# TakiRyo/object-triggered-3D-SLAM

Measured on AMD Instinct MI355X. Metric: RGB-D frames/sec (640×480, 5mm voxel TSDF) at 1/2/4/8 GPU; Mpoints/s filtered, higher is better.
Workload: dtype f32 tsdf/weight + f64 colour; 1 GPU; configs[1]: 256-frame 640x480 RGB-D TSDF integration, 5 mm voxel, sdf_trunc 0.04, one object scan per GPU (synthetic box-on-floor ring scan), colour precision 64 (Open3D's float64 TSDFVoxel::color_, exact division: bit-exact colours); color_precision=64, width=640, height=480, volume_units=5896, parallelism=objects1

## Files before the change

object-triggered-3d-slam_amd/_lib.py:

```python
from __future__ import annotations

import ctypes as C
import os
import threading

_HERE = os.path.dirname(os.path.abspath(__file__))
LIB_PATH = os.path.join(_HERE, "libotslam_hip.so")
HEADER_PATH = os.path.join(os.path.dirname(_HERE), "include", "otslam.h")

OT_OK = 0
OT_ERR_INVALID_ARGUMENT = 1
OT_ERR_UNSUPPORTED_FORMAT = 2
OT_ERR_CAPACITY = 3
OT_ERR_HIP = 4

OT_COLOR_NONE = 0
OT_COLOR_RGB8 = 1


class ot_intrinsics(C.Structure):
    _fields_ = [("width", C.c_int32), ("height", C.c_int32), ("fx", C.c_double), ("fy", C.c_double),
                ("cx", C.c_double), ("cy", C.c_double)]


# ... 123 lines not shown
class OTError(RuntimeError):
    """Raised for any non-OK status; message mirrors Open3D's utility::LogError text."""


TEST_SIGNATURES = {
    "otx_serial_chain_f64": [_p, _i64, _i32, _p, _pi64, _p],
    "otx_chain_walk_trace": [_p, _i64, _i32, _p, _p, _i32, _p],
    "otx_tsdf_stats": [_p, _p],
    "otx_unit_sort_radix": [_i32],
    "otx_sor_netfill": [_i32],
    "otx_integrate_fine": [_i32],
    "otx_integrate_workgroup": [_i32],
    "otx_touch_stage_blocks": [_i32],
    "otx_touch_frames": [_i32],
    "otx_split_frontend": [_i32],
    "otx_defer_integrate": [_i32],
    "otx_integrate_depth": [_i32],
    "otx_mc_emit_fork": [_i32],
    "otx_normals_at": [_i32],
    "otx_sampler_hi_stream": [_i32],
    "otx_sort_pairs_u64_u32": [_p, _p, _p, _p, _i64, _i32, _p],
    "otx_sort_segments_u32_u32": [_p, _p, _p, _p, _p, _i32, _i32, _p],
    "otx_alloc_count": [],
    "otx_registration_last_d2": [_p, _i64, _p],
}


def use_variant(path: str) -> None:
    global LIB_PATH
    path = os.path.abspath(path)
# ... 66 lines not shown
```

object-triggered-3d-slam_amd/csrc/tsdf.h:

```cpp
#pragma once

#include <vector>

#include "common.h"

namespace ot {

constexpr int UNIT_RES = 16;
constexpr int UNIT_VOX = UNIT_RES * UNIT_RES * UNIT_RES;
constexpr int UNIT_FIELDS = 5;
constexpr int UNIT_FLOATS = UNIT_FIELDS * UNIT_VOX;
constexpr int UNIT_FLOATS_C64 = 8 * UNIT_VOX;

constexpr int C_UNUSED0 = 0;
constexpr int C_UNITS = 1;
constexpr int C_OVERFLOW = 2;
constexpr int C_HASHERR = 3;
constexpr int C_BATCH_PAIRS = 4;
constexpr int C_ORDER_HEAVY = 6;
constexpr int C_ORDER_LIGHT = 7;
constexpr int C_KMAX = 8;
constexpr int C_KNEG = 11;
constexpr int C_UNITS_DONE = 14;
constexpr int N_COUNTERS = 16;

constexpr int S_UPDATES = 0;
constexpr int S_UNIT_INTEGRATIONS = 1;

struct TsdfDev {
    unsigned long long* hkeys;
    int* hvals;
    int* counters;
    unsigned long long* stats;
    int* unit_keys;
    float* vox;
    int unit_floats;
    int color64;
    unsigned long long* fmask;
    int* bslots;
    void* work;
    int hash_mask;
    int max_units;
// ... 110 lines not shown
};

struct IntegrateParams {
    const float* depth;
    const uint8_t* color;
    const float* mult;
    int W, H;
    float fx, fy, cx, cy;
    float E[12];
    float es0, es1, es2;
    float vl, half, trunc, trunc_inv, safe_w, safe_h;
    float inv_fx, inv_fy;
    float proj_eps;
    int rcp_hi;
    double unit_len;
};

struct BatchTouchParams {
    int W, stride, ws, hs;
    double fx, fy, cx, cy;
    double trunc, unit_len;
    double inv_unit;
    int slot_cap;
    int64_t npx;
    int pc;
    int tiles;
    int stage_blocks;
    int tf;
    int sample_stage;
};

struct StageMaskParams {
    int W, H, tiles_x, tiles_y, wpr;
    float fx, fy, cx, cy, vl, half;
    double unit_len;
    int nframes;
};

struct UnitWork {
    int id;
    int kx, ky, kz;
    unsigned long long mask;
    unsigned long long pad;
};

enum class BatchMode { Direct, Overlap, Deferred };
struct BatchPlan {
    BatchMode mode = BatchMode::Direct;
    bool split = false;
    int set = 0;
    int* wcount = nullptr;
    int* wcopy = nullptr;
};

struct BatchCtx {
    BatchPlan plan;
    BatchTouchParams tp;
    IntegrateParams ip0;
    StageMaskParams sq{};
    unsigned* smask = nullptr;
    int n, pc, variant;
};

struct PendingFrame {
// ... 47 lines not shown
    ot_intrinsics mult_intr{};
    bool mult_valid = false;
    int batch_max = ot::MAX_BATCH;
    std::vector<ot::PendingFrame> pending;
    ot::BatchFrame* hbframes = nullptr;
    unsigned* hmail = nullptr;
    int hb_next = 0;
    unsigned units_seq = 0;
    int early_frame = -1;
    unsigned mc_seq = 0;
    int batch_pc = ot::C_BATCH_PAIRS;
    struct BatchSet {
        ot::BatchFrame* bframes = nullptr;
        uint2* bdc = nullptr;
        int64_t cap = 0;
        void* work = nullptr;
        hipEvent_t ev_units = nullptr;
        hipEvent_t ev_done = nullptr;
    } bset[2];
    int overlap_mode = -1;
    unsigned* tmask = nullptr;
    int64_t tmask_words = 0;
    int tmask_w = 0, tmask_h = 0;
    int split_mode = -1;
    bool dfr_on = false;
    hipStream_t dfr_stream = nullptr;
    hipEvent_t ev_dfr = nullptr;
    ot::BatchCtx dfr;
    int64_t stat_batches = 0, stat_unit_batches = 0, stat_fresh = 0, stat_prev_units = 0;
    int64_t last_batch_slots = -1;
// ... 18 lines not shown
    std::vector<std::pair<hipEvent_t, hipEvent_t>> prof_fe_events;
    double prof_fe_ms = 0.0;
    int64_t prof_fe_batches = 0;
};

namespace ot {
struct TsdfHooks {
    int int_fine = -1;
    int fine_units = -1;
    int int_depth = -1;
    int int_wg = -1;
    int stage_blocks = -1;
    int touch_tf = -1;
    int split = -1;
    int defer = -1;
    bool unit_sort_radix = false;
};
extern TsdfHooks g_tsdf_hooks;

ot_status reserve_units(ot_tsdf* vol, int64_t extra, hipStream_t stream);
ot_status export_list(ot_tsdf* vol, hipStream_t stream, const unsigned** ids, int64_t* n);
ot_status tsdf_sorted_units(ot_tsdf* vol, hipStream_t stream, int64_t* n_units);
struct MailSrc {
    const unsigned* p[ot::OT_MAIL_WORDS];
    int n;
};
ot_status mail_words(ot_tsdf* vol, const MailSrc& s, hipStream_t stream);
ot_status mail_wait(const unsigned* word, unsigned seq, hipStream_t stream);
ot_status tsdf_flush(ot_tsdf* vol, hipStream_t stream, bool join = true);
ot_status wait_normals(ot_tsdf* vol, hipStream_t stream);
// ... 6 lines not shown
```

object-triggered-3d-slam_amd/csrc/tsdf.hip:

```cpp
#include <algorithm>
#include <cmath>
#include <cstring>
#include <type_traits>
#include <utility>

#include "tsdf.h"

namespace ot {

typedef unsigned u32x2 __attribute__((ext_vector_type(2)));

__device__ inline __amdgpu_buffer_rsrc_t make_rsrc(const void* base, int bytes) {
    return __builtin_amdgcn_make_buffer_rsrc(const_cast<void*>(base), (short)0, bytes, 0x00020000);
}

__device__ inline double ld_f64(__amdgpu_buffer_rsrc_t r, int i) {
    const u32x2 v = __builtin_amdgcn_raw_buffer_load_b64(r, i * 8, 0, 0);
    return __hiloint2double((int)v.y, (int)v.x);
}
__device__ inline void st_f64(__amdgpu_buffer_rsrc_t r, int i, double x) {
    u32x2 v;
    v.x = (unsigned)__double2loint(x);
    v.y = (unsigned)__double2hiint(x);
    __builtin_amdgcn_raw_buffer_store_b64(v, r, i * 8, 0, 0);
}
// ... 129 lines not shown
        unsigned long long k = keys[h];
        if (k == KEY_EMPTY) {
            const unsigned long long old = atomicCAS(&keys[h], KEY_EMPTY, key);
            if (old == KEY_EMPTY) used[atomicAdd(nused, 1)] = (unsigned short)h;
            k = (old == KEY_EMPTY) ? key : old;
        }
        if (k == key) {
            atomicOr(&masks[h], bit);
            return true;
        }
        h = (h + 1) & (LTAB - 1);
    }
    return false;
}

__device__ inline void stage_share(const BatchFrame* __restrict__ frames, const BatchTouchParams& p, int nframes,
                                   int grp, int part, int parts) {
    const int64_t quads = (p.npx + 3) >> 2;
    const int64_t per = (quads + parts - 1) / parts;
    const int64_t q0 = (int64_t)part * per, q1 = q0 + per < quads ? q0 + per : quads;
    for (int f = grp * p.tf; f < grp * p.tf + p.tf && f < nframes; ++f)
        prep_range(frames[f], q0 + threadIdx.x, q1, p.npx);
}

struct TouchLds {
    unsigned long long keys[LTAB];
    unsigned long long masks[LTAB];
    unsigned short used[LTAB];
    int nused;
};
template <bool REPLAY, bool STAGE = !REPLAY>
__device__ __forceinline__ void touch_body(const BatchFrame* __restrict__ frames, const BatchTouchParams& p,
                                           const TsdfDev& d, int nframes, TouchLds& L, int tile, int grp) {
    unsigned long long* s_keys = L.keys;
    unsigned long long* s_masks = L.masks;
    unsigned short* s_used = L.used;
    int& s_nused = L.nused;
// ... 552 lines not shown
        frame_tap<ZB, true>(fr, p, npx, fpx, fpy, fpz, z0, pixv, pcz, dv, cv);
        bool some = false;
#pragma unroll
        for (int k = 0; k < ZB; ++k) some |= cand[k] = voxel_candidate<true>(p, pixv[k], pcz[k], dv[k], df[k]);
        if (__builtin_amdgcn_ballot_w64(some) == 0ull) continue;
        const __amdgpu_buffer_rsrc_t mult_rsrc = make_rsrc(p.mult, npx * 4);
#pragma unroll
        for (int k = 0; k < ZB; ++k) mv[k] = voxel_multiplier<true>(mult_rsrc, pixv[k], cand[k]);
#pragma unroll
        for (int k = 0; k < ZB; ++k)
            voxel_update<C64, FAST>(cand[k], df[k] * __uint_as_float(mv[k]), cv[k], use_color, p, s_r32, s_r64, ts[k],
                                    wt[k], cr[k], cg[k], cb[k], upd);
    }
}

template <bool C64, bool FAST, int ZB, int KT>
__device__ __forceinline__ void integrate_item(const BatchFrame* __restrict__ frames, const IntegrateParams& p,
                                               const TsdfDev& d, const UnitWork& w, int s, int npx,
                                               const float* s_r32, const double* s_r64, unsigned& upd) {
    using CT = typename std::conditional<C64, double, float>::type;
    const int ent = w.id;
    const unsigned long long mask = w.mask;
    if (ent == -1) return;
    const int id = ent & 0x7FFFFFFF;
    const bool fresh = ent < 0;
    unsigned tid = threadIdx.x;
    asm volatile("" : "+v"(tid));
    const int lane = tid & 63;
    const int x = (s & 2) * 4 + (lane >> 3), y = (s & 1) * 8 + (lane & 7);
    const int col = x * 16 + y;
    const int z0 = (s >> 2) * ZB;
    float* base = d.vox + (size_t)id * (C64 ? UNIT_FLOATS_C64 : UNIT_FLOATS);
    const __amdgpu_buffer_rsrc_t col64 = make_rsrc(base + 2 * UNIT_VOX, 3 * UNIT_VOX * 8);
    float ts[ZB], wt[ZB];
    CT cr[ZB], cg[ZB], cb[ZB];
#pragma unroll
    for (int k = 0; k < ZB; ++k) {
// ... 90 lines not shown
            st_f64(col64, UNIT_VOX + vi, cg[k]);
            st_f64(col64, 2 * UNIT_VOX + vi, cb[k]);
        } else {
            base[2 * UNIT_VOX + vi] = cr[k];
            base[3 * UNIT_VOX + vi] = cg[k];
            base[4 * UNIT_VOX + vi] = cb[k];
        }
    }
}

template <bool C64, bool FAST>
struct RcpLds {
    float r32[(FAST && !C64) ? RCP_N + 1 : 1];
    double r64[(FAST && C64) ? RCP_N + 1 : 1];
};
template <bool C64, bool FAST, int ZB, int KT, bool HEAVY, int WG>
__device__ __forceinline__ void integrate_body(const BatchFrame* __restrict__ frames, const IntegrateParams& p,
                                               const TsdfDev& d, const UnitWork* __restrict__ work,
                                               const int* __restrict__ wcount, float* s_r32, double* s_r64, int bid,
                                               int nblk) {
    constexpr int PARTS = 4 * (UNIT_RES / ZB) / WG;
    {
        const int n0 = __builtin_amdgcn_readfirstlane(__hip_atomic_load(wcount, __ATOMIC_RELAXED, __HIP_MEMORY_SCOPE_AGENT));
        if (bid >= (PARTS == 1 ? n0 : ((n0 + 7) / 8) * 8 * PARTS)) return;
    }
    if constexpr (FAST) {
        for (int r = 1 + threadIdx.x; r <= p.rcp_hi; r += 64 * WG) {
            if constexpr (C64) s_r64[r] = 1.0 / (double)r;
            else s_r32[r] = 1.0f / (float)r;
        }
        if constexpr (WG > 1) __syncthreads();
        else __builtin_amdgcn_fence(__ATOMIC_ACQ_REL, "wavefront");
    }
    const int wave = __builtin_amdgcn_readfirstlane((int)(threadIdx.x >> 6));
    const int n = *wcount;
    const int nh = HEAVY ? wcount[2] : 0;
    const int npx = p.W * p.H;
    unsigned upd = 0;
    const int items = PARTS == 1 ? n : ((n + 7) / 8) * 8 * PARTS;
    for (int it = bid; it < items; it += nblk) {
        const int u = PARTS == 1 ? it : (it / (8 * PARTS)) * 8 + (it & 7);
        if (PARTS > 1 && u >= n) continue;
        const int part = PARTS == 1 ? 0 : (it >> 3) % PARTS;
        const int s = part * WG + wave;
        integrate_item<C64, FAST, ZB, KT>(frames, p, d, work[!HEAVY || u < nh ? u : n - 1 - (u - nh)], s, npx, s_r32,
                                          s_r64, upd);
    }
    const unsigned long long tot = wave_sum((unsigned long long)upd);
    if ((threadIdx.x & 63) == 0 && tot) atomicAdd(&d.stats[S_UPDATES], tot);
}

extern __shared__ double s_rcp_dyn[];
template <bool C64, bool FAST, int ZB = BZ, int KT = 1, int WG = INT_WG>
__global__ __launch_bounds__(64 * WG, (C64 && !FAST) ? 5 : (ZB == 2 ? 4 : INT_WAVES_PER_EU)) void k_batch_integrate(
    const BatchFrame* __restrict__ frames, IntegrateParams p, TsdfDev d, const UnitWork* __restrict__ work,
    const int* __restrict__ wcount) {
    integrate_body<C64, FAST, ZB, KT, false, WG>(frames, p, d, work, wcount, reinterpret_cast<float*>(s_rcp_dyn),
                                                 s_rcp_dyn, (int)blockIdx.x, (int)gridDim.x);
}

template <bool C64, bool FAST>
__global__ __launch_bounds__(64 * INT_WG, (C64 && !FAST) ? 5 : INT_WAVES_PER_EU) void k_integrate_touch(
    const BatchFrame* __restrict__ frames, IntegrateParams p, TsdfDev d, const UnitWork* __restrict__ work,
    const int* __restrict__ wcount, int nint, const BatchFrame* __restrict__ tframes, BatchTouchParams tp, int tn) {
    union Lds {
        TouchLds t;
        RcpLds<C64, FAST> r;
    };
    __shared__ Lds lds;
    const int b = (int)blockIdx.x;
    if (b < nint) {
        integrate_body<C64, FAST, BZ, 1, true, INT_WG>(frames, p, d, work, wcount, lds.r.r32, lds.r.r64, b, nint);
    } else {
// ... 37 lines not shown
    for (int k = 0; k < 16; ++k) E[k] = (float)ext[k];
    for (int k = 0; k < 12; ++k) p.E[k] = E[k];
    const double unit_voxel_length = vol->unit_length / (double)UNIT_RES;
    p.vl = (float)unit_voxel_length;
    p.half = p.vl * 0.5f;
    p.es0 = E[0 * 4 + 2] * p.vl;
    p.es1 = E[1 * 4 + 2] * p.vl;
    p.es2 = E[2 * 4 + 2] * p.vl;
    p.trunc = (float)vol->sdf_trunc;
    p.trunc_inv = 1.0f / p.trunc;
    p.safe_w = (float)in->width - 0.0001f;
    p.safe_h = (float)in->height - 0.0001f;
    p.proj_eps = (float)(std::ldexp((double)std::max(in->width, in->height) + 2.0, -21) + 1.2e-4);
    p.rcp_hi = RCP_N;
    p.unit_len = vol->unit_length;
    return p;
}

static ot_status launch_deferred(ot_tsdf* vol, hipStream_t stream, const BatchCtx* next);
static ot_status ensure_mult(ot_tsdf* vol, const ot_intrinsics* in, hipStream_t stream) {
    if (vol->mult_valid && std::memcmp(&vol->mult_intr, in, sizeof(ot_intrinsics)) == 0) return OT_OK;
    if (vol->mult) {
        ot_status sd = launch_deferred(vol, stream, nullptr);
        if (sd != OT_OK) return sd;
        if (vol->istream) OT_HIP_TRY(hipStreamSynchronize(vol->istream));
        OT_HIP_TRY(hipStreamSynchronize(stream));
        OT_HIP_TRY(hipFree(vol->mult));
        vol->mult = nullptr;
    }
    OT_HIP_TRY(hipMalloc(&vol->mult, sizeof(float) * (size_t)in->width * in->height));
// ... 240 lines not shown
    OT_HIP_TRY(hipStreamSynchronize(stream));
    for (void* p : {(void*)d.vox, (void*)d.unit_keys, (void*)vol->sorted_ids, (void*)d.hkeys, (void*)d.hvals,
                    (void*)d.fmask, (void*)d.bslots, d.work, vol->bset[1].work})
        if (p) (void)hipFree(p);
    d = nd;
    vol->bset[1].work = work1;
    vol->sorted_ids = nsorted;
    vol->max_units = nmax;
    vol->hash_cap = cap;
    return OT_OK;
}


static ot_status plan_batch(ot_tsdf* vol, const ot_intrinsics& in, int pc, BatchPlan& p) {
    p.split = split_on(vol) && tmask_fits(in.width, in.height);
    p.mode = defer_on(vol, p.split) ? BatchMode::Deferred : overlap_on(vol) ? BatchMode::Overlap : BatchMode::Direct;
    p.wcount = vol->dev.counters + pc;
    if (p.mode != BatchMode::Direct) {
        ot_status st = ensure_overlap(vol);
        if (st != OT_OK) return st;
        p.set = vol->bset_next;
        vol->bset_next ^= 1;
        p.wcount = p.wcopy = vol->wcount + p.set;
    }
    return OT_OK;
}

static void fill_batch_frames(const ot_tsdf* vol, const PendingFrame* frames, int n, uint2* bdc, int64_t npx, float vl,
                              BatchFrame* host) {
    for (int k = 0; k < n; ++k) {
// ... 19 lines not shown
    BatchTouchParams tp;
    tp.npx = (int64_t)in.width * in.height;
    tp.pc = pc;
    tp.W = in.width, tp.stride = vol->stride;
    tp.ws = (in.width + vol->stride - 1) / vol->stride;
    tp.hs = (in.height + vol->stride - 1) / vol->stride;
    tp.fx = in.fx, tp.fy = in.fy, tp.cx = in.cx, tp.cy = in.cy;
    tp.trunc = vol->sdf_trunc;
    tp.unit_len = vol->unit_length, tp.inv_unit = 1.0 / vol->unit_length;
    tp.slot_cap = (int)vol->hash_cap;
    tp.tiles = ((tp.ws + TT - 1) / TT) * ((tp.hs + TT - 1) / TT);
    tp.stage_blocks = g_tsdf_hooks.stage_blocks < 0 ? 2 * tp.tiles : g_tsdf_hooks.stage_blocks;
    tp.tf = g_tsdf_hooks.touch_tf > 0 ? g_tsdf_hooks.touch_tf : TF;
    tp.sample_stage = split ? 1 : 0;
    if (split) tp.stage_blocks = -1;
    return tp;
}

static StageMaskParams make_stage_params(const ot_tsdf* vol, const ot_intrinsics& in, const IntegrateParams& ip, int n) {
    StageMaskParams q;
    q.W = in.width, q.H = in.height;
    q.tiles_x = (in.width + STX - 1) / STX;
    q.tiles_y = (in.height + STY - 1) / STY;
    q.wpr = (q.tiles_x + 31) / 32;
    q.fx = ip.fx, q.fy = ip.fy, q.cx = ip.cx, q.cy = ip.cy;
    q.vl = ip.vl, q.half = ip.half;
    q.unit_len = vol->unit_length;
    q.nframes = n;
    return q;
}
// ... 153 lines not shown
            if (vol->istream) OT_HIP_TRY(hipStreamSynchronize(vol->istream));
            OT_HIP_TRY(hipFree(bs.bdc));
            bs.bdc = nullptr;
        }
        const int64_t cap = npx * std::max(n, std::min(vol->batch_max, MAX_BATCH));
        OT_HIP_TRY(hipMalloc(&bs.bdc, sizeof(uint2) * cap));
        bs.cap = cap;
    }
    BatchFrame* host = vol->hbframes + vol->hb_next * MAX_BATCH;
    vol->hb_next ^= 1;
    bc.ip0 = make_integrate_params(vol, nullptr, nullptr, vol->mult, &in, frames[0].extrinsic);
    fill_batch_frames(vol, frames, n, bs.bdc, npx, bc.ip0.vl, host);
    hipLaunchKernelGGL(k_copy_frames, dim3(1), dim3(COPY_FRAMES_LANES), 0, stream, (const uint4*)host,
                       (uint4*)bs.bframes, (int)(sizeof(BatchFrame) / 16) * n);
    bc.tp = make_touch_params(vol, in, bc.pc, plan.split);
    if (plan.split) {
        if ((st = ensure_tmask(vol, in.width, in.height, stream)) != OT_OK) return st;
        bc.sq = make_stage_params(vol, in, bc.ip0, n);
        bc.smask = vol->tmask;
    }
    const bool fast = !vol->imported && (int64_t)vol->frame_id + n < RCP_N;
    bc.variant = (vol->color64 ? 2 : 0) + (fast ? 1 : 0);
    bc.ip0.rcp_hi = (int)std::min<int64_t>((int64_t)vol->frame_id + n, RCP_N);
    if (plan.mode != BatchMode::Deferred) bc.variant = slice_form(bc.variant, direct_estimate(vol), false);

    ProfPair fe;
    if ((st = prof_open(vol, fe, stream)) != OT_OK) return st;
    const bool fused = plan.mode == BatchMode::Deferred && vol->dfr_on;
    if (fused && (st = launch_deferred(vol, stream, &bc)) != OT_OK) return st;
    launch_front_end(vol, bc, false, !fused, stream);
// ... 131 lines not shown
```

object-triggered-3d-slam_amd/csrc/tsdf_volume.hip:

```cpp
#include <algorithm>
#include <chrono>
#include <cmath>
#include <cstring>
#include <sched.h>
#include <thread>

#include "tsdf.h"

namespace ot {

TsdfHooks g_tsdf_hooks;

static void reset_host_state(ot_tsdf* v) {
    v->batch_pc = C_BATCH_PAIRS;
    v->frame_id = 0;
    v->imported = false;
    v->early_frame = -1;
    v->last_batch_slots = -1;
    v->stat_batches = v->stat_unit_batches = v->stat_fresh = v->stat_prev_units = 0;
    v->sorted_frame = -1;
    v->sorted_units = -1;
    v->mesh.nv = v->mesh.nt = 0;
    v->mesh.valid = false;
    v->cloud.valid = false;
// ... 41 lines not shown
            if (q != hipErrorNotReady) OT_HIP_TRY(q);
        }
        if (now < t_sleep) sched_yield();
        else std::this_thread::sleep_for(std::chrono::microseconds(20));
    }
}

__global__ __launch_bounds__(256) void k_tsdf_clear(TsdfDev d, int64_t cap) {
    for (int64_t i = (int64_t)blockIdx.x * 256 + threadIdx.x; i < cap; i += (int64_t)gridDim.x * 256) {
        d.hkeys[i] = ~0ull;
        d.hvals[i] = -1;
        d.fmask[i] = 0ull;
    }
    if (blockIdx.x == 0) {
        if (threadIdx.x < N_COUNTERS) d.counters[threadIdx.x] = 0;
        if (threadIdx.x < 4) d.stats[threadIdx.x] = 0ull;
    }
}

}

using namespace ot;

extern "C" {

ot_status ot_tsdf_create(double voxel_length, double sdf_trunc, int32_t color_type, int32_t unit_res, int32_t stride,
                         int64_t max_units, ot_tsdf** out) {
    if (!out) return fail(OT_ERR_INVALID_ARGUMENT, "[ScalableTSDFVolume] out is NULL");
    *out = nullptr;
    if (!(voxel_length > 0.0) || !(sdf_trunc > 0.0))
        return fail(OT_ERR_INVALID_ARGUMENT, "[ScalableTSDFVolume] voxel_length and sdf_trunc must be positive");
// ... 15 lines not shown
    int64_t cap = 1;
    while (cap < 4 * max_units) cap <<= 1;
    v->hash_cap = cap;
    TsdfDev& d = v->dev;
    d.hash_mask = (int)(cap - 1);
    d.max_units = (int)max_units;
    auto cleanup = [&](hipError_t e) {
        set_error(std::string("[ScalableTSDFVolume] allocation failed: ") + hipGetErrorString(e));
        ot_tsdf_destroy(v);
        return OT_ERR_HIP;
    };
    hipError_t e;
    if ((e = hipMalloc(&d.hkeys, sizeof(unsigned long long) * cap)) != hipSuccess) return cleanup(e);
    if ((e = hipMalloc(&d.hvals, sizeof(int) * cap)) != hipSuccess) return cleanup(e);
    if ((e = hipMalloc(&d.counters, sizeof(int) * N_COUNTERS)) != hipSuccess) return cleanup(e);
    if ((e = hipMalloc(&d.stats, sizeof(unsigned long long) * 4)) != hipSuccess) return cleanup(e);
    if ((e = hipMalloc(&d.unit_keys, sizeof(int) * 3 * max_units)) != hipSuccess) return cleanup(e);
    v->color64 = color_type == OT_COLOR_RGB8;
    d.color64 = v->color64 ? 1 : 0;
    d.unit_floats = v->color64 ? UNIT_FLOATS_C64 : UNIT_FLOATS;
    if ((e = hipMalloc(&d.vox, sizeof(float) * (size_t)d.unit_floats * max_units)) != hipSuccess) return cleanup(e);
    if ((e = hipMalloc(&v->sorted_ids, sizeof(unsigned) * max_units)) != hipSuccess) return cleanup(e);
    if ((e = hipMalloc(&d.fmask, sizeof(unsigned long long) * cap)) != hipSuccess) return cleanup(e);
    if ((e = hipMalloc(&d.bslots, sizeof(int) * cap)) != hipSuccess) return cleanup(e);
    if ((e = hipMalloc(&d.work, sizeof(UnitWork) * cap)) != hipSuccess) return cleanup(e);
    if ((e = hipMalloc(&v->bset[0].bframes, sizeof(BatchFrame) * MAX_BATCH)) != hipSuccess) return cleanup(e);
    if ((e = hipHostMalloc(&v->hbframes, sizeof(BatchFrame) * MAX_BATCH * 2, hipHostMallocCoherent)) != hipSuccess)
        return cleanup(e);
    if ((e = hipHostMalloc(&v->hmail, sizeof(unsigned) * 2 * OT_MAIL_WORDS, hipHostMallocCoherent)) != hipSuccess)
        return cleanup(e);
    std::memset(v->hmail, 0, sizeof(unsigned) * 2 * OT_MAIL_WORDS);
// ... 2 lines not shown
        ot_tsdf_destroy(v);
        return st;
    }
    *out = v;
    return OT_OK;
}

ot_status ot_tsdf_destroy(ot_tsdf* v) {
    if (!v) return OT_OK;
    (void)hipDeviceSynchronize();
    TsdfDev& d = v->dev;
    ot_tsdf_set_profiling(v, 0);
    void* ptrs[] = {d.hkeys, d.hvals, d.counters, d.stats, d.unit_keys, d.vox, v->mult, v->sorted_ids, v->mesh.ws,
                    v->mesh.v, v->mesh.c, v->mesh.t, v->mesh.vk, v->mesh.tk, v->mesh.vown, d.fmask, d.bslots, d.work,
                    v->cloud.ws, v->wcount, v->bset[0].bframes, v->bset[0].bdc, v->bset[1].bframes, v->bset[1].bdc,
                    v->bset[1].work, v->tmask};
    for (void* p : ptrs)
        if (p) (void)hipFree(p);
    if (v->hbframes) (void)hipHostFree(v->hbframes);
    if (v->hmail) (void)hipHostFree(v->hmail);
    if (v->ev_fork) (void)hipEventDestroy(v->ev_fork);
    if (v->ev_join) (void)hipEventDestroy(v->ev_join);
    if (v->ev_normals) (void)hipEventDestroy(v->ev_normals);
    if (v->ev_made) (void)hipEventDestroy(v->ev_made);
    if (v->ev_dfr) (void)hipEventDestroy(v->ev_dfr);
    if (v->side) (void)hipStreamDestroy(v->side);
    if (v->istream) (void)hipStreamDestroy(v->istream);
    for (auto& b : v->bset) {
        if (b.ev_units) (void)hipEventDestroy(b.ev_units);
        if (b.ev_done) (void)hipEventDestroy(b.ev_done);
    }
    delete v;
    return OT_OK;
}

ot_status ot_tsdf_reset(ot_tsdf* v) {
    if (!v) return fail(OT_ERR_INVALID_ARGUMENT, "[ScalableTSDFVolume::Reset] volume is NULL");
    TsdfDev& d = v->dev;
    OT_HIP_TRY(hipDeviceSynchronize());
    v->normals_pending = false;
    v->last_set = -1;
    OT_HIP_TRY(hipMemset(d.hkeys, 0xFF, sizeof(unsigned long long) * v->hash_cap));
    OT_HIP_TRY(hipMemset(d.hvals, 0xFF, sizeof(int) * v->hash_cap));
    OT_HIP_TRY(hipMemset(d.fmask, 0, sizeof(unsigned long long) * v->hash_cap));
    OT_HIP_TRY(hipMemset(d.counters, 0, sizeof(int) * N_COUNTERS));
    OT_HIP_TRY(hipMemset(d.stats, 0, sizeof(unsigned long long) * 4));
    OT_HIP_TRY(hipDeviceSynchronize());
    v->pending.clear();
    v->dfr_on = false;
    reset_host_state(v);
    return OT_OK;
}

ot_status ot_tsdf_reset_async(ot_tsdf* v, void* stream_) {
    if (!v) return fail(OT_ERR_INVALID_ARGUMENT, "[ScalableTSDFVolume::Reset] volume is NULL");
    hipStream_t stream = S(stream_);
    ot_status st = tsdf_flush(v, stream);
    if (st != OT_OK) return st;
    st = wait_normals(v, stream);
    if (st != OT_OK) return st;
    const unsigned blocks = (unsigned)std::min<int64_t>((v->hash_cap + 255) / 256, 2048);
// ... 44 lines not shown
}

ot_status ot_tsdf_batch_stats(ot_tsdf* vol, int64_t* batches, int64_t* unit_batches, int64_t* new_units) {
    if (!vol) return fail(OT_ERR_INVALID_ARGUMENT, "invalid arguments");
    if (batches) *batches = vol->stat_batches;
    if (unit_batches) *unit_batches = vol->stat_unit_batches;
    if (new_units) *new_units = vol->stat_fresh;
    return OT_OK;
}

ot_status ot_tsdf_counters(ot_tsdf* vol, int64_t* updates, int64_t* unit_integrations, void* stream_) {
    if (!vol) return fail(OT_ERR_INVALID_ARGUMENT, "invalid arguments");
    hipStream_t stream = S(stream_);
    ot_status st = tsdf_flush(vol, stream);
    if (st != OT_OK) return st;
    unsigned long long s[4];
    OT_HIP_TRY(hipMemcpyAsync(s, vol->dev.stats, sizeof(s), hipMemcpyDeviceToHost, stream));
    OT_HIP_TRY(hipStreamSynchronize(stream));
    if (updates) *updates = (int64_t)s[S_UPDATES];
    if (unit_integrations) *unit_integrations = (int64_t)s[S_UNIT_INTEGRATIONS];
    return OT_OK;
}

ot_status ot_tsdf_set_color_precision(ot_tsdf* vol, int32_t bits) {
    if (!vol || (bits != 32 && bits != 64))
        return fail(OT_ERR_INVALID_ARGUMENT, "[ScalableTSDFVolume] colour precision must be 32 or 64 bits");
    int nu = 0;
    OT_HIP_TRY(hipMemcpy(&nu, vol->dev.counters + C_UNITS, sizeof(int), hipMemcpyDeviceToHost));
    if (nu != 0 || !vol->pending.empty())
        return fail(OT_ERR_INVALID_ARGUMENT, "[ScalableTSDFVolume] set the colour precision before the first integrate");
    const bool c64 = bits == 64 && vol->color_type == OT_COLOR_RGB8;
    if (c64 != vol->color64) {
        const int uf = c64 ? UNIT_FLOATS_C64 : UNIT_FLOATS;
// ... 56 lines not shown

ot_status ot_tsdf_frontend_time(ot_tsdf* vol, double* total_ms, int64_t* batches) {
    if (!vol) return fail(OT_ERR_INVALID_ARGUMENT, "invalid arguments");
    ot_status st = tsdf_flush(vol, nullptr);
    if (st != OT_OK) return st;
    if ((st = drain_events(vol->prof_fe_events, vol->prof_fe_ms, vol->prof_fe_batches)) != OT_OK) return st;
    if (total_ms) *total_ms = vol->prof_fe_ms;
    if (batches) *batches = vol->prof_fe_batches;
    return OT_OK;
}

ot_status otx_tsdf_stats(ot_tsdf* vol, uint64_t* out4) {
    if (!vol || !out4) return fail(OT_ERR_INVALID_ARGUMENT, "invalid arguments");
    ot_status st = tsdf_flush(vol, nullptr);
    if (st != OT_OK) return st;
    OT_HIP_TRY(hipMemcpy(out4, vol->dev.stats, sizeof(uint64_t) * 4, hipMemcpyDeviceToHost));
    return OT_OK;
}

ot_status otx_integrate_fine(int32_t mode) {
    g_tsdf_hooks.int_fine = mode < 0 ? -1 : (mode == 1 ? 1 : 0);
    g_tsdf_hooks.fine_units = mode >= 2 ? mode : -1;
    return OT_OK;
}

ot_status otx_integrate_workgroup(int32_t waves) {
    if (waves != -1 && waves != 1 && waves != 2 && waves != 4)
        return fail(OT_ERR_INVALID_ARGUMENT, "otx_integrate_workgroup: -1, 1, 2 or 4 waves");
    g_tsdf_hooks.int_wg = waves;
    return OT_OK;
}
// ... 43 lines not shown
    return OT_OK;
}

ot_status otx_integrate_depth(int32_t kt) {
    if (kt != -1 && (kt < 1 || kt > 3)) return fail(OT_ERR_INVALID_ARGUMENT, "integrate pipeline depth must be -1 or 1..3");
    g_tsdf_hooks.int_depth = kt;
    return OT_OK;
}

ot_status otx_defer_integrate(int32_t mode) {
    if (mode < -1 || mode > 1) return fail(OT_ERR_INVALID_ARGUMENT, "deferred integrate mode must be -1, 0 or 1");
    g_tsdf_hooks.defer = mode;
    return OT_OK;
}

ot_status otx_split_frontend(int32_t mode) {
    if (mode < -1 || mode > 1) return fail(OT_ERR_INVALID_ARGUMENT, "split front end mode must be -1, 0 or 1");
    g_tsdf_hooks.split = mode;
    return OT_OK;
}

ot_status ot_tsdf_set_shard_block(ot_tsdf* vol, int32_t log2_units) {
    if (!vol || log2_units < 0 || log2_units > 8)
        return fail(OT_ERR_INVALID_ARGUMENT, "[ScalableTSDFVolume] shard block must be 2^0 .. 2^8 units per axis");
    int nu = 0;
    OT_HIP_TRY(hipMemcpy(&nu, vol->dev.counters + C_UNITS, sizeof(int), hipMemcpyDeviceToHost));
    if (nu != 0 || !vol->pending.empty())
        return fail(OT_ERR_INVALID_ARGUMENT, "[ScalableTSDFVolume] set the shard before the first integrate");
    vol->dev.shard_shift = log2_units;
    return OT_OK;
// ... 4 lines not shown
```

Measured before the change: 90510 frames/s.

## Add per-tile depth max map and conservative slice pretest to skip idle frames

```diff
diff --git a/object-triggered-3d-slam_amd/_lib.py b/object-triggered-3d-slam_amd/_lib.py
--- a/object-triggered-3d-slam_amd/_lib.py
+++ b/object-triggered-3d-slam_amd/_lib.py
@@ -161,6 +161,7 @@
     "otx_touch_stage_blocks": [_i32],
     "otx_touch_frames": [_i32],
     "otx_split_frontend": [_i32],
+    "otx_slice_pretest": [_i32],
     "otx_defer_integrate": [_i32],
     "otx_integrate_depth": [_i32],
     "otx_mc_emit_fork": [_i32],
diff --git a/object-triggered-3d-slam_amd/csrc/slice_pretest.h b/object-triggered-3d-slam_amd/csrc/slice_pretest.h
--- /dev/null
+++ b/object-triggered-3d-slam_amd/csrc/slice_pretest.h
@@ -0,0 +1,103 @@
+#pragma once
+
+#include <math.h>
+#include <stdint.h>
+
+#if defined(__HIPCC__) || defined(__CUDACC__)
+#define OT_PRE_HD __host__ __device__ inline
+#else
+#define OT_PRE_HD inline
+#endif
+
+namespace ot {
+
+constexpr int PRE_TILE = 8;
+constexpr int PRE_CAP = 4;
+constexpr int PRE_NONE = 1 << 28;
+constexpr int PRE_SLACK = 8;
+constexpr float PRE_Z_GUARD = 0.01f;
+constexpr float PRE_PAD_ABS = 1e-4f;
+constexpr float PRE_PAD_REL = 3.814697265625e-06f;
+
+struct PreTile4 {
+    uint32_t k[4];
+};
+
+struct PreIntrinsics {
+    int W, H;
+    float fx, fy, cx, cy;
+};
+
+OT_PRE_HD int pre_tiles(int n) { return (n + PRE_TILE - 1) / PRE_TILE; }
+
+OT_PRE_HD uint32_t pre_depth_key(float d) {
+    uint32_t b = 0u;
+    if (d > 0.0f) __builtin_memcpy(&b, &d, 4);
+    return b;
+}
+
+template <class TileFn>
+OT_PRE_HD bool slice_idle(const float* E, const PreIntrinsics& in, float vl, double unit_len, int kx, int ky, int kz,
+                          int s, float trunc, TileFn&& tile4) {
+    const float half = vl * 0.5f;
+    const int x0 = (s & 2) * 4, y0 = (s & 1) * 8, z0 = (s >> 2) * 4;
+    const float o[3] = {(float)((double)kx * unit_len), (float)((double)ky * unit_len), (float)((double)kz * unit_len)};
+    const float lo[3] = {half + vl * (float)x0 + o[0], half + vl * (float)y0 + o[1], half + vl * (float)z0 + o[2]};
+    const float vl2 = vl + vl, vl3 = vl2 + vl, vl7 = (vl2 + vl2) + vl3;
+    const float ext[3] = {vl7, vl7, vl3};
+    const float mid[3] = {lo[0] + 0.5f * ext[0], lo[1] + 0.5f * ext[1], lo[2] + 0.5f * ext[2]};
+    const float far_[3] = {fabsf(lo[0]) + ext[0], fabsf(lo[1]) + ext[1], fabsf(half + o[2]) + 32.0f * vl};
+    float bl[3], bh[3];
+    for (int a = 0; a < 3; ++a) {
+        const float e0 = E[a * 4 + 0], e1 = E[a * 4 + 1], e2 = E[a * 4 + 2], t = E[a * 4 + 3];
+        const float a0 = fabsf(e0), a1 = fabsf(e1), a2 = fabsf(e2);
+        const float c = e0 * mid[0] + e1 * mid[1] + e2 * mid[2] + t;
+        const float r = 0.5f * (a0 * ext[0] + a1 * ext[1] + a2 * ext[2]);
+        const float m = a0 * far_[0] + a1 * far_[1] + a2 * far_[2] + fabsf(t);
+        const float pad = r + (PRE_PAD_ABS + PRE_PAD_REL * m);
+        bl[a] = c - pad, bh[a] = c + pad;
+    }
+    const float zl = bl[2], zh = bh[2];
+    if (!(zl > PRE_Z_GUARD) || !(zh < 1e30f)) return false;
+    const float izl = 1.0f / zl, izh = 1.0f / zh;
+    const float xl = in.fx * bl[0], xh = in.fx * bh[0], yl = in.fy * bl[1], yh = in.fy * bh[1];
+    const float ua = xl * izl, ub = xl * izh, uc = xh * izl, ud = xh * izh;
+    const float va = yl * izl, vb = yl * izh, vc = yh * izl, vd = yh * izh;
+    float umin = fminf(fminf(ua, ub), fminf(uc, ud)) + (in.cx + 0.5f);
+    float umax = fmaxf(fmaxf(ua, ub), fmaxf(uc, ud)) + (in.cx + 0.5f);
+    float vmin = fminf(fminf(va, vb), fminf(vc, vd)) + (in.cy + 0.5f);
+    float vmax = fmaxf(fmaxf(va, vb), fmaxf(vc, vd)) + (in.cy + 0.5f);
+    if (!(umin <= umax) || !(vmin <= vmax)) return false;
+    const float W = (float)in.W, H = (float)in.H;
+    const float wide = 0.01f + 9.5367431640625e-07f * (W > H ? W : H);
+    umin = fmaxf(umin - wide, -4.0f), umax = fminf(umax + wide, W + 4.0f);
+    vmin = fmaxf(vmin - wide, -4.0f), vmax = fminf(vmax + wide, H + 4.0f);
+    int u0 = (int)floorf(umin) - 1, u1 = (int)floorf(umax) + 1;
+    int v0 = (int)floorf(vmin) - 1, v1 = (int)floorf(vmax) + 1;
+    if (u1 < 0 || v1 < 0 || u0 > in.W - 1 || v0 > in.H - 1 || u0 > u1 || v0 > v1) return true;
+    u0 = u0 < 0 ? 0 : u0, v0 = v0 < 0 ? 0 : v0;
+    u1 = u1 > in.W - 1 ? in.W - 1 : u1, v1 = v1 > in.H - 1 ? in.H - 1 : v1;
+    const int tx0 = u0 / PRE_TILE, tx1 = u1 / PRE_TILE, ty0 = v0 / PRE_TILE, ty1 = v1 / PRE_TILE;
+    if (tx1 - tx0 >= PRE_CAP || ty1 - ty0 >= PRE_CAP) return false;
+    const int tmx = pre_tiles(in.W);
+    PreTile4 q[PRE_CAP];
+#if defined(__HIP_DEVICE_COMPILE__)
+#pragma unroll
+#endif
+    for (int r = 0; r < PRE_CAP; ++r)
+        q[r] = tile4(ty0 + r <= ty1 ? (ty0 + r) * tmx + tx0 : PRE_NONE);
+    const int last = tx1 - tx0;
+    uint32_t best = 0u;
+    for (int j = 0; j < 4; ++j) {
+        uint32_t k = 0u;
+        for (int r = 0; r < PRE_CAP; ++r) k = q[r].k[j] > k ? q[r].k[j] : k;
+        k = j <= last ? k : 0u;
+        best = k > best ? k : best;
+    }
+    if (best == 0u) return true;
+    float D;
+    __builtin_memcpy(&D, &best, 4);
+    return D - zl <= -trunc;
+}
+
+}
diff --git a/object-triggered-3d-slam_amd/csrc/tsdf.h b/object-triggered-3d-slam_amd/csrc/tsdf.h
--- a/object-triggered-3d-slam_amd/csrc/tsdf.h
+++ b/object-triggered-3d-slam_amd/csrc/tsdf.h
@@ -26,6 +26,10 @@
 
 constexpr int S_UPDATES = 0;
 constexpr int S_UNIT_INTEGRATIONS = 1;
+constexpr int S_PRETEST_DROPPED = 2;
+constexpr int S_DROP_BASE = 8, S_DROP_LINES = 256, S_DROP_STRIDE = 8;
+constexpr int S_UPD_BASE = S_DROP_BASE + S_DROP_LINES * S_DROP_STRIDE;
+constexpr int N_STATS = S_UPD_BASE + S_DROP_LINES * S_DROP_STRIDE;
 
 struct TsdfDev {
     unsigned long long* hkeys;
@@ -166,6 +170,9 @@
     float proj_eps;
     int rcp_hi;
     double unit_len;
+    const unsigned* tmax;
+    int tmax_tiles;
+    int tmax_words;
 };
 
 struct BatchTouchParams {
@@ -180,6 +187,8 @@
     int stage_blocks;
     int tf;
     int sample_stage;
+    unsigned* tmax;
+    int H;
 };
 
 struct StageMaskParams {
@@ -200,6 +209,7 @@
 struct BatchPlan {
     BatchMode mode = BatchMode::Direct;
     bool split = false;
+    bool pretest = false;
     int set = 0;
     int* wcount = nullptr;
     int* wcopy = nullptr;
@@ -277,6 +287,8 @@
         ot::BatchFrame* bframes = nullptr;
         uint2* bdc = nullptr;
         int64_t cap = 0;
+        unsigned* tmax = nullptr;
+        int64_t tmax_cap = 0;
         void* work = nullptr;
         hipEvent_t ev_units = nullptr;
         hipEvent_t ev_done = nullptr;
@@ -325,6 +337,7 @@
     int touch_tf = -1;
     int split = -1;
     int defer = -1;
+    int pretest = -1;
     bool unit_sort_radix = false;
 };
 extern TsdfHooks g_tsdf_hooks;
diff --git a/object-triggered-3d-slam_amd/csrc/tsdf.hip b/object-triggered-3d-slam_amd/csrc/tsdf.hip
--- a/object-triggered-3d-slam_amd/csrc/tsdf.hip
+++ b/object-triggered-3d-slam_amd/csrc/tsdf.hip
@@ -4,11 +4,13 @@
 #include <type_traits>
 #include <utility>
 
+#include "slice_pretest.h"
 #include "tsdf.h"
 
 namespace ot {
 
 typedef unsigned u32x2 __attribute__((ext_vector_type(2)));
+typedef unsigned u32x4 __attribute__((ext_vector_type(4)));
 
 __device__ inline __amdgpu_buffer_rsrc_t make_rsrc(const void* base, int bytes) {
     return __builtin_amdgcn_make_buffer_rsrc(const_cast<void*>(base), (short)0, bytes, 0x00020000);
@@ -168,13 +170,58 @@
     return false;
 }
 
+__device__ inline unsigned group8_max(unsigned v) {
+    v = max(v, (unsigned)__shfl_xor((int)v, 1));
+    v = max(v, (unsigned)__shfl_xor((int)v, 2));
+    return max(v, (unsigned)__shfl_xor((int)v, 4));
+}
+__device__ __noinline__ void tile_max_range(const BatchFrame& fr, unsigned* __restrict__ map, int W, int H, int i0,
+                                            int step) {
+    const int tmx = pre_tiles(W), total = tmx * pre_tiles(H) * PRE_TILE;
+    const bool rows16 = fr.depth16 && (W & 7) == 0 && (reinterpret_cast<uintptr_t>(fr.depth16) & 15) == 0;
+    for (int i = i0; i < total; i += step) {
+        const int t = i >> 3, y = (t / tmx) * PRE_TILE + (i & 7), x0 = (t % tmx) * PRE_TILE;
+        const int cols = min(PRE_TILE, W - x0);
+        const bool inside = y < H;
+        unsigned key = 0u;
+        bool done = false;
+        if (rows16) {
+            unsigned m = 0u;
+            if (inside) {
+                const uint4 v = *reinterpret_cast<const uint4*>(fr.depth16 + (int64_t)y * W + x0);
+                const unsigned w4[4] = {v.x, v.y, v.z, v.w};
+#pragma unroll
+                for (int k = 0; k < 4; ++k) m = max(m, max(w4[k] & 0xFFFFu, w4[k] >> 16));
+            }
+            m = group8_max(m);
+            const float d = prep_depth(fr, m);
+            done = m == 0u || d > 0.0f;
+            key = pre_depth_key(d);
+        }
+        if (!done) {
+            key = 0u;
+            if (inside)
+                for (int c = 0; c < cols; ++c) {
+                    const int64_t px = (int64_t)y * W + x0 + c;
+                    key = max(key, pre_depth_key(fr.depth16 ? prep_depth(fr, fr.depth16[px]) : fr.depthf[px]));
+                }
+            key = group8_max(key);
+        }
+        if ((i & 7) == 0) map[t] = key;
+    }
+}
+
 __device__ inline void stage_share(const BatchFrame* __restrict__ frames, const BatchTouchParams& p, int nframes,
                                    int grp, int part, int parts) {
     const int64_t quads = (p.npx + 3) >> 2;
     const int64_t per = (quads + parts - 1) / parts;
     const int64_t q0 = (int64_t)part * per, q1 = q0 + per < quads ? q0 + per : quads;
-    for (int f = grp * p.tf; f < grp * p.tf + p.tf && f < nframes; ++f)
+    for (int f = grp * p.tf; f < grp * p.tf + p.tf && f < nframes; ++f) {
         prep_range(frames[f], q0 + threadIdx.x, q1, p.npx);
+        if (p.tmax)
+            tile_max_range(frames[f], p.tmax + (size_t)f * (pre_tiles(p.W) * pre_tiles(p.H)), p.W, p.H,
+                           part * 256 + (int)threadIdx.x, parts * 256);
+    }
 }
 
 struct TouchLds {
@@ -757,13 +804,38 @@
     }
 }
 
+__device__ __forceinline__ unsigned long long pretest_idle(const BatchFrame* __restrict__ frames,
+                                                           const IntegrateParams& p, const UnitWork& w, int s,
+                                                           unsigned long long mask) {
+    unsigned tid = threadIdx.x;
+    asm volatile("" : "+v"(tid));
+    const int f = (int)(tid & 63u);
+    bool idle = false;
+    PreIntrinsics in;
+    in.W = p.W, in.H = p.H, in.fx = p.fx, in.fy = p.fy, in.cx = p.cx, in.cy = p.cy;
+    float vl = p.vl, trunc = p.trunc;
+    double unit_len = p.unit_len;
+    asm volatile("" : "+s"(in.fx), "+s"(in.fy), "+s"(in.cx), "+s"(in.cy), "+s"(vl), "+s"(trunc), "+s"(unit_len));
+    asm volatile("" : "+s"(in.W), "+s"(in.H));
+    if ((mask >> f) & 1ull) {
+        const __amdgpu_buffer_rsrc_t map = make_rsrc(p.tmax, (p.tmax_words + PRE_SLACK) * 4);
+        const int base = f * p.tmax_tiles;
+        idle = slice_idle(frames[f].E, in, vl, unit_len, w.kx, w.ky, w.kz, s, trunc, [&](int i) {
+            const u32x4 v = __builtin_amdgcn_raw_buffer_load_b128(map, (base + i) * 4, 0, 0);
+            PreTile4 q;
+            q.k[0] = v.x, q.k[1] = v.y, q.k[2] = v.z, q.k[3] = v.w;
+            return q;
+        });
+    }
+    return __builtin_amdgcn_ballot_w64(idle);
+}
+
 template <bool C64, bool FAST, int ZB, int KT>
 __device__ __forceinline__ void integrate_item(const BatchFrame* __restrict__ frames, const IntegrateParams& p,
-                                               const TsdfDev& d, const UnitWork& w, int s, int npx,
-                                               const float* s_r32, const double* s_r64, unsigned& upd) {
+                                               const TsdfDev& d, const UnitWork& w, unsigned long long mask, int s,
+                                               int npx, const float* s_r32, const double* s_r64, unsigned& upd) {
     using CT = typename std::conditional<C64, double, float>::type;
     const int ent = w.id;
-    const unsigned long long mask = w.mask;
     if (ent == -1) return;
     const int id = ent & 0x7FFFFFFF;
     const bool fresh = ent < 0;
@@ -884,7 +956,7 @@
     float r32[(FAST && !C64) ? RCP_N + 1 : 1];
     double r64[(FAST && C64) ? RCP_N + 1 : 1];
 };
-template <bool C64, bool FAST, int ZB, int KT, bool HEAVY, int WG>
+template <bool C64, bool FAST, int ZB, int KT, bool HEAVY, int WG, bool PRE = false>
 __device__ __forceinline__ void integrate_body(const BatchFrame* __restrict__ frames, const IntegrateParams& p,
                                                const TsdfDev& d, const UnitWork* __restrict__ work,
                                                const int* __restrict__ wcount, float* s_r32, double* s_r64, int bid,
@@ -907,17 +979,32 @@
     const int nh = HEAVY ? wcount[2] : 0;
     const int npx = p.W * p.H;
     unsigned upd = 0;
+    unsigned dropped = 0;
     const int items = PARTS == 1 ? n : ((n + 7) / 8) * 8 * PARTS;
     for (int it = bid; it < items; it += nblk) {
         const int u = PARTS == 1 ? it : (it / (8 * PARTS)) * 8 + (it & 7);
         if (PARTS > 1 && u >= n) continue;
         const int part = PARTS == 1 ? 0 : (it >> 3) % PARTS;
         const int s = part * WG + wave;
-        integrate_item<C64, FAST, ZB, KT>(frames, p, d, work[!HEAVY || u < nh ? u : n - 1 - (u - nh)], s, npx, s_r32,
-                                          s_r64, upd);
+        const UnitWork& w = work[!HEAVY || u < nh ? u : n - 1 - (u - nh)];
+        unsigned long long mask = w.mask;
+        if constexpr (PRE) {
+            if (p.tmax && w.id != -1) {
+                const unsigned long long idle = pretest_idle(frames, p, w, s, mask);
+                mask &= ~idle;
+                dropped += (unsigned)__popcll(idle);
+                if (!mask && w.id >= 0) continue;
+            }
+        }
+        integrate_item<C64, FAST, ZB, KT>(frames, p, d, w, mask, s, npx, s_r32, s_r64, upd);
     }
     const unsigned long long tot = wave_sum((unsigned long long)upd);
-    if ((threadIdx.x & 63) == 0 && tot) atomicAdd(&d.stats[S_UPDATES], tot);
+    if ((threadIdx.x & 63) == 0 && tot)
+        atomicAdd(&d.stats[S_UPD_BASE + (bid & (S_DROP_LINES - 1)) * S_DROP_STRIDE], tot);
+    if constexpr (PRE) {
+        if ((threadIdx.x & 63) == 0 && dropped)
+            atomicAdd(&d.stats[S_DROP_BASE + (bid & (S_DROP_LINES - 1)) * S_DROP_STRIDE], (unsigned long long)dropped);
+    }
 }
 
 extern __shared__ double s_rcp_dyn[];
@@ -925,8 +1012,9 @@
 __global__ __launch_bounds__(64 * WG, (C64 && !FAST) ? 5 : (ZB == 2 ? 4 : INT_WAVES_PER_EU)) void k_batch_integrate(
     const BatchFrame* __restrict__ frames, IntegrateParams p, TsdfDev d, const UnitWork* __restrict__ work,
     const int* __restrict__ wcount) {
-    integrate_body<C64, FAST, ZB, KT, false, WG>(frames, p, d, work, wcount, reinterpret_cast<float*>(s_rcp_dyn),
-                                                 s_rcp_dyn, (int)blockIdx.x, (int)gridDim.x);
+    integrate_body<C64, FAST, ZB, KT, false, WG, ZB == BZ>(frames, p, d, work, wcount,
+                                                           reinterpret_cast<float*>(s_rcp_dyn), s_rcp_dyn,
+                                                           (int)blockIdx.x, (int)gridDim.x);
 }
 
 template <bool C64, bool FAST>
@@ -994,6 +1082,8 @@
     p.proj_eps = (float)(std::ldexp((double)std::max(in->width, in->height) + 2.0, -21) + 1.2e-4);
     p.rcp_hi = RCP_N;
     p.unit_len = vol->unit_length;
+    p.tmax = nullptr;
+    p.tmax_tiles = p.tmax_words = 0;
     return p;
 }
 
@@ -1264,6 +1354,9 @@
 
 static ot_status plan_batch(ot_tsdf* vol, const ot_intrinsics& in, int pc, BatchPlan& p) {
     p.split = split_on(vol) && tmask_fits(in.width, in.height);
+    const int pre = g_tsdf_hooks.pretest;
+    p.pretest = !p.split && (pre > 0 || (pre < 0 && vol->dev.shard_world <= 1)) &&
+                (int64_t)pre_tiles(in.width) * pre_tiles(in.height) * MAX_BATCH + PRE_SLACK < (int64_t)PRE_NONE;
     p.mode = defer_on(vol, p.split) ? BatchMode::Deferred : overlap_on(vol) ? BatchMode::Overlap : BatchMode::Direct;
     p.wcount = vol->dev.counters + pc;
     if (p.mode != BatchMode::Direct) {
@@ -1313,6 +1406,8 @@
     tp.tf = g_tsdf_hooks.touch_tf > 0 ? g_tsdf_hooks.touch_tf : TF;
     tp.sample_stage = split ? 1 : 0;
     if (split) tp.stage_blocks = -1;
+    tp.tmax = nullptr;
+    tp.H = in.height;
     return tp;
 }
 
@@ -1496,6 +1591,24 @@
     hipLaunchKernelGGL(k_copy_frames, dim3(1), dim3(COPY_FRAMES_LANES), 0, stream, (const uint4*)host,
                        (uint4*)bs.bframes, (int)(sizeof(BatchFrame) / 16) * n);
     bc.tp = make_touch_params(vol, in, bc.pc, plan.split);
+    if (plan.pretest) {
+        const int64_t tiles = (int64_t)pre_tiles(in.width) * pre_tiles(in.height);
+        if (bs.tmax_cap < tiles * n) {
+            if (bs.tmax) {
+                OT_HIP_TRY(hipStreamSynchronize(stream));
+                if (vol->istream) OT_HIP_TRY(hipStreamSynchronize(vol->istream));
+                OT_HIP_TRY(hipFree(bs.tmax));
+                bs.tmax = nullptr, bs.tmax_cap = 0;
+            }
+            const int64_t cap = tiles * std::max(n, std::min(vol->batch_max, MAX_BATCH));
+            OT_HIP_TRY(hipMalloc(&bs.tmax, sizeof(unsigned) * (cap + PRE_SLACK)));
+            bs.tmax_cap = cap;
+        }
+        bc.tp.tmax = bs.tmax;
+        bc.ip0.tmax = bs.tmax;
+        bc.ip0.tmax_tiles = (int)tiles;
+        bc.ip0.tmax_words = (int)(tiles * n);
+    }
     if (plan.split) {
         if ((st = ensure_tmask(vol, in.width, in.height, stream)) != OT_OK) return st;
         bc.sq = make_stage_params(vol, in, bc.ip0, n);
diff --git a/object-triggered-3d-slam_amd/csrc/tsdf_volume.hip b/object-triggered-3d-slam_amd/csrc/tsdf_volume.hip
--- a/object-triggered-3d-slam_amd/csrc/tsdf_volume.hip
+++ b/object-triggered-3d-slam_amd/csrc/tsdf_volume.hip
@@ -79,7 +79,7 @@
     }
     if (blockIdx.x == 0) {
         if (threadIdx.x < N_COUNTERS) d.counters[threadIdx.x] = 0;
-        if (threadIdx.x < 4) d.stats[threadIdx.x] = 0ull;
+        for (int i = threadIdx.x; i < N_STATS; i += 256) d.stats[i] = 0ull;
     }
 }
 
@@ -125,7 +125,7 @@
     if ((e = hipMalloc(&d.hkeys, sizeof(unsigned long long) * cap)) != hipSuccess) return cleanup(e);
     if ((e = hipMalloc(&d.hvals, sizeof(int) * cap)) != hipSuccess) return cleanup(e);
     if ((e = hipMalloc(&d.counters, sizeof(int) * N_COUNTERS)) != hipSuccess) return cleanup(e);
-    if ((e = hipMalloc(&d.stats, sizeof(unsigned long long) * 4)) != hipSuccess) return cleanup(e);
+    if ((e = hipMalloc(&d.stats, sizeof(unsigned long long) * N_STATS)) != hipSuccess) return cleanup(e);
     if ((e = hipMalloc(&d.unit_keys, sizeof(int) * 3 * max_units)) != hipSuccess) return cleanup(e);
     v->color64 = color_type == OT_COLOR_RGB8;
     d.color64 = v->color64 ? 1 : 0;
@@ -158,7 +158,7 @@
     void* ptrs[] = {d.hkeys, d.hvals, d.counters, d.stats, d.unit_keys, d.vox, v->mult, v->sorted_ids, v->mesh.ws,
                     v->mesh.v, v->mesh.c, v->mesh.t, v->mesh.vk, v->mesh.tk, v->mesh.vown, d.fmask, d.bslots, d.work,
                     v->cloud.ws, v->wcount, v->bset[0].bframes, v->bset[0].bdc, v->bset[1].bframes, v->bset[1].bdc,
-                    v->bset[1].work, v->tmask};
+                    v->bset[1].work, v->tmask, v->bset[0].tmax, v->bset[1].tmax};
     for (void* p : ptrs)
         if (p) (void)hipFree(p);
     if (v->hbframes) (void)hipHostFree(v->hbframes);
@@ -188,7 +188,7 @@
     OT_HIP_TRY(hipMemset(d.hvals, 0xFF, sizeof(int) * v->hash_cap));
     OT_HIP_TRY(hipMemset(d.fmask, 0, sizeof(unsigned long long) * v->hash_cap));
     OT_HIP_TRY(hipMemset(d.counters, 0, sizeof(int) * N_COUNTERS));
-    OT_HIP_TRY(hipMemset(d.stats, 0, sizeof(unsigned long long) * 4));
+    OT_HIP_TRY(hipMemset(d.stats, 0, sizeof(unsigned long long) * N_STATS));
     OT_HIP_TRY(hipDeviceSynchronize());
     v->pending.clear();
     v->dfr_on = false;
@@ -263,9 +263,11 @@
     hipStream_t stream = S(stream_);
     ot_status st = tsdf_flush(vol, stream);
     if (st != OT_OK) return st;
-    unsigned long long s[4];
-    OT_HIP_TRY(hipMemcpyAsync(s, vol->dev.stats, sizeof(s), hipMemcpyDeviceToHost, stream));
+    std::vector<unsigned long long> s(N_STATS);
+    OT_HIP_TRY(hipMemcpyAsync(s.data(), vol->dev.stats, sizeof(unsigned long long) * N_STATS, hipMemcpyDeviceToHost,
+                              stream));
     OT_HIP_TRY(hipStreamSynchronize(stream));
+    for (int i = 0; i < S_DROP_LINES; ++i) s[S_UPDATES] += s[S_UPD_BASE + i * S_DROP_STRIDE];
     if (updates) *updates = (int64_t)s[S_UPDATES];
     if (unit_integrations) *unit_integrations = (int64_t)s[S_UNIT_INTEGRATIONS];
     return OT_OK;
@@ -352,7 +354,13 @@
     if (!vol || !out4) return fail(OT_ERR_INVALID_ARGUMENT, "invalid arguments");
     ot_status st = tsdf_flush(vol, nullptr);
     if (st != OT_OK) return st;
-    OT_HIP_TRY(hipMemcpy(out4, vol->dev.stats, sizeof(uint64_t) * 4, hipMemcpyDeviceToHost));
+    std::vector<unsigned long long> s(N_STATS);
+    OT_HIP_TRY(hipMemcpy(s.data(), vol->dev.stats, sizeof(unsigned long long) * N_STATS, hipMemcpyDeviceToHost));
+    for (int i = 0; i < 4; ++i) out4[i] = s[i];
+    for (int i = 0; i < S_DROP_LINES; ++i) {
+        out4[S_PRETEST_DROPPED] += s[S_DROP_BASE + i * S_DROP_STRIDE];
+        out4[S_UPDATES] += s[S_UPD_BASE + i * S_DROP_STRIDE];
+    }
     return OT_OK;
 }
 
@@ -426,6 +434,12 @@
     return OT_OK;
 }
 
+ot_status otx_slice_pretest(int32_t mode) {
+    if (mode < -1 || mode > 1) return fail(OT_ERR_INVALID_ARGUMENT, "slice pre-test mode must be -1, 0 or 1");
+    g_tsdf_hooks.pretest = mode;
+    return OT_OK;
+}
+
 ot_status otx_split_frontend(int32_t mode) {
     if (mode < -1 || mode > 1) return fail(OT_ERR_INVALID_ARGUMENT, "split front end mode must be -1, 0 or 1");
     g_tsdf_hooks.split = mode;
```

After: 95980 frames/s (median of 6 runs). 1.06x the previous value.
